# zhuker/lamejs

Measured on NVIDIA H100. Metric: encoded audio seconds/sec (44.1kHz stereo 128kbps CBR), higher is better.
Workload: dtype f64

## Files before the change

### lamejs_b200/csrc/k_quant.cuh

```cuda
#ifndef MP3B200_K_QUANT_CUH
#define MP3B200_K_QUANT_CUH
#include <stddef.h>
#include "mp3_device.cuh"
#include "mp3_tables.h"
#include "k_psy.cuh"

#define Q_LARGE_BITS 100000
#define Q_IXMAX 8206
#define Q_FULL 0xffffffffu

struct GranuleInfoDev {
  int global_gain, part2_3_length, part2_length, big_values, count1, scalefac_compress;
  int table_select[3], region0_count, region1_count, preflag, scalefac_scale, count1table_select, block_type;
  int subblock_gain[4];
  int count1bits, sfbmax, sfbdivide, sfb_lmax, psymax, psy_lmax, sfb_smin, max_nonzero_coeff;
  int scalefac[MP3_SFBMAX];
  int slen[4];
  int part_row;
  int pad_;
  double xrpow_max;
};
struct QuantFrameState {
  int stream, rel_frame;
  int in_old[2], in_step[2];
// ... 868 lines not shown
#pragma unroll 1
    for (int i = 0; i < MP3_SFBMAX; i++) gi->scalefac[i] = 0;
    gi->xrpow_max = 0;
  }
  const Mp3Geo* geo = &T->geo[is_short ? 1 : 0];
  if (lane == 0) wk->geo = geo;
  {
    float4 v[5];
#pragma unroll
    for (int k = 0; k < 5; k++) { const int q = lane + 32 * k; if (q < 144) v[k] = __ldg(reinterpret_cast<const float4*>(xr_g) + q); }
    if (!is_short) {
#pragma unroll
      for (int k = 0; k < 5; k++) { const int q = lane + 32 * k; if (q < 144) reinterpret_cast<float4*>(wk->xr)[q] = v[k]; }
    } else {
#pragma unroll
      for (int k = 0; k < 5; k++) {
        const int q = lane + 32 * k;
        if (q < 144) {
          const short* ro = geo->reorder + 4 * q;
          wk->xr[__ldg(ro + 0)] = v[k].x; wk->xr[__ldg(ro + 1)] = v[k].y; wk->xr[__ldg(ro + 2)] = v[k].z; wk->xr[__ldg(ro + 3)] = v[k].w;
        }
      }
    }
  }
  __syncwarp();
  if (!is_short) {
    const int lo = T->psfb21[0];
    const double lf = (double)T->longfact[21];
    int keep = lo - 1;
#pragma unroll 1
    for (int j = lo + lane; j < 576; j += 32) {
      int g = 0;
      while (g < 5 && j >= T->psfb21[g + 1]) g++;
      double ath21 = ath_ps[g];
      if (lf > 1e-12) ath21 *= lf;
      if (!(fabs((double)wk->xr[j]) < ath21)) keep = j;
    }
    keep = wmax(keep);
    __syncwarp();
#pragma unroll 1
    for (int j = keep + 1 + lane; j < 576; j += 32) wk->xr[j] = 0.0f;
  } else if (lane == 0) {
#pragma unroll 1
    for (int block = 0; block < 3; block++) {
      bool stop = false;
#pragma unroll 1
      for (int g = 5; g >= 0 && !stop; g--) {
        const int start = T->sfb_s[12] * 3 + (T->sfb_s[13] - T->sfb_s[12]) * block + (T->psfb12[g] - T->psfb12[0]);
        const int end = start + (T->psfb12[g + 1] - T->psfb12[g]);
        double ath12 = ath_ps[g];
        if ((double)T->shortfact[12] > 1e-12) ath12 *= (double)T->shortfact[12];
#pragma unroll 1
        for (int j = end - 1; j >= start; j--) {
          if (fabs((double)wk->xr[j]) < ath12) wk->xr[j] = 0.0f;
          else { stop = true; break; }
        }
      }
    }
  }
  __syncwarp();
  {
    float mx = 0.0f, amax = 0.0f;
#pragma unroll 1
    for (int p = lane; p < 288; p += 32) {
      const float2 x = *reinterpret_cast<const float2*>(&wk->xr[2 * p]);
      const double t0 = fabs((double)x.x), t1 = fabs((double)x.y);
      f32s p0, p1; p0 = sqrt(t0 * sqrt(t0)); p1 = sqrt(t1 * sqrt(t1));
      float2 o; o.x = p0.v; o.y = p1.v;
      *reinterpret_cast<float2*>(&wk->xrpow[2 * p]) = o;
      mx = fmaxf(mx, fmaxf(p0.v, p1.v));
      amax = fmaxf(amax, fmaxf((float)t0, (float)t1));
    }
#pragma unroll 1
    for (int o = 16; o > 0; o >>= 1) { mx = fmaxf(mx, __shfl_xor_sync(Q_FULL, mx, o)); amax = fmaxf(amax, __shfl_xor_sync(Q_FULL, amax, o)); }
    bool energy;
    if ((double)amax > 1E-20) energy = true;
    else {
      if (lane == 0) { double sum = 0; for (int i = 0; i <= 575; ++i) sum += fabs((double)wk->xr[i]); wk->scratch[1] = sum > 1E-20; }
      __syncwarp();
      energy = wk->scratch[1] != 0;
      __syncwarp();
    }
    if (lane == 0) gi->xrpow_max = (double)mx;
    __syncwarp();
    if (!energy) {
#pragma unroll 1
      for (int i = lane; i < 576; i += 32) wk->ixw[i] = 0;
      __syncwarp();
      return false;
    }
  }
  const double masking_lower = is_short ? T->masking_lower_short : T->masking_lower_long;
  if (!is_short) {
    if (need_xmin && lane < 21) {
      const int gsfb = lane;
      int j = T->sfb_l[gsfb];
      const int width = wk->geo->width[gsfb];
      double xmin = ath_adjust * (double)T->ath_l[gsfb];
      double en0 = 0.0;
#pragma unroll 1
      for (int l = width >> 1; l > 0; l--) {
        double xa = (double)wk->xr[j] * (double)wk->xr[j]; en0 += xa; j++;
        double xb = (double)wk->xr[j] * (double)wk->xr[j]; en0 += xb; j++;
      }
      const double e = (double)ratio->en_l[gsfb];
      if (e > 0.0) {
        const double x = en0 * (double)ratio->thm_l[gsfb] * masking_lower / e;
        if (xmin < x) xmin = x;
      }
      f32s o; o = xmin * (double)T->longfact[gsfb];
      wk->xmin[gsfb] = o.v;
    }
    int last = -1;
#pragma unroll 1
    for (int i = lane; i < 576; i += 32) if (wk->xr[i] != 0.0f) last = i;
    last = wmax(last);
    int mnz = last + 1;
    if (mnz > 575) mnz = 575;
    if (lane == 0) gi->max_nonzero_coeff = mnz;
  } else {
#pragma unroll 1
    for (int t = lane; need_xmin && t < 36; t += 32) {
      const int sfb = t / 3, b = t - 3 * sfb;
      const int width = wk->geo->width[t];
      int j = 3 * T->sfb_s[sfb] + b * width;
      const double tmpATH = ath_adjust * (double)T->ath_s[sfb];
      double en0 = 0.0;
#pragma unroll 1
      for (int l = width >> 1; l > 0; l--) {
        double xa = (double)wk->xr[j] * (double)wk->xr[j]; en0 += xa; j++;
        double xb = (double)wk->xr[j] * (double)wk->xr[j]; en0 += xb; j++;
      }
      double xmin = tmpATH;
      const double e = (double)ratio->en_s[sfb][b];
      if (e > 0.0) {
        const double x = en0 * (double)ratio->thm_s[sfb][b] * masking_lower / e;
        if (xmin < x) xmin = x;
      }
      f32s o; o = xmin * (double)T->shortfact[sfb];
      wk->xmin[t] = o.v;
    }
    __syncwarp();
    if (need_xmin && lane < 12) {
      f32s* p = reinterpret_cast<f32s*>(&wk->xmin[3 * lane]);
      if ((double)p[0] > (double)p[1]) p[1] += ((double)p[0] - (double)p[1]) * T->decay;
      if ((double)p[1] > (double)p[2]) p[2] += ((double)p[1] - (double)p[2]) * T->decay;
    }
    if (lane == 0) gi->max_nonzero_coeff = 575;
  }
  __syncwarp();
  return true;
}

__device__ __noinline__ void best_scalefac_store_w(GcWork* wk, int* scfsi, const GranuleInfoDev* __restrict__ g0, int gr, int mode_gr) {
  const int lane = LANE;
  GranuleInfoDev* gi = &wk->b;
#pragma unroll 1
  for (int s0 = 0; s0 < gi->sfbmax; s0 += 32) {
    const int sfb = s0 + lane;
    if (sfb < gi->sfbmax) {
      const int j = wk->geo->start[sfb];
      bool any = false;
#pragma unroll 1
      for (int l = 0; l < wk->geo->width[sfb]; l += 2) if (*reinterpret_cast<const unsigned*>(&wk->ixw[j + l]) != 0) { any = true; break; }
      wk->mode[sfb] = any ? 1 : 0;
    }
  }
  __syncwarp();
  const int sfbmax = gi->sfbmax;
  int recalc_w = 0;
  {
    bool z = false;
#pragma unroll 1
    for (int sfb = lane; sfb < sfbmax; sfb += 32) if (!wk->mode[sfb]) { gi->scalefac[sfb] = -2; z = true; }
    if (__any_sync(Q_FULL, z)) recalc_w = -2;
  }
  __syncwarp();
  if (0 == gi->scalefac_scale && 0 == gi->preflag) {
    int sor = 0;
#pragma unroll 1
    for (int sfb = lane; sfb < sfbmax; sfb += 32) { const int v = gi->scalefac[sfb]; if (v > 0) sor |= v; }
    sor = (int)__reduce_or_sync(Q_FULL, (unsigned)sor);
    if (0 == (sor & 1) && sor != 0) {
#pragma unroll 1
      for (int sfb = lane; sfb < sfbmax; sfb += 32) { const int v = gi->scalefac[sfb]; if (v > 0) gi->scalefac[sfb] = v >> 1; }
      __syncwarp();
      if (lane == 0) gi->scalefac_scale = 1;
      recalc_w = 1;
    }
  }
  __syncwarp();
  if (0 == gi->preflag && gi->block_type != BT_SHORT && mode_gr == 2) {
    const bool in = lane >= 11 && lane < 21;
    const int v = in ? gi->scalefac[lane] : 0, pt = pretab_of(lane);
    const bool ok = !in || !(v < pt && v != -2);
    if (__all_sync(Q_FULL, ok)) {
      if (in && v > 0) gi->scalefac[lane] = v - pt;
      __syncwarp();
      if (lane == 0) gi->preflag = 1;
      recalc_w = 1;
    }
  }
  __syncwarp();
  if (lane == 0) {
    int recalc = recalc_w;
#pragma unroll 1
    for (int i = 0; i < 4; i++) scfsi[i] = 0;
    if (gr == 1 && g0->block_type != BT_SHORT && gi->block_type != BT_SHORT) {
      const int* g0sf = g0->scalefac;
      const int band[5] = {0, 6, 11, 16, 21};
      int sfb;
#pragma unroll 1
      for (int i = 0; i < 4; i++) {
#pragma unroll 1
        for (sfb = band[i]; sfb < band[i + 1]; sfb++)
          if (g0sf[sfb] != gi->scalefac[sfb] && gi->scalefac[sfb] >= 0) break;
        if (sfb == band[i + 1]) {
#pragma unroll 1
          for (sfb = band[i]; sfb < band[i + 1]; sfb++) gi->scalefac[sfb] = -1;
          scfsi[i] = 1;
        }
      }
      int s1 = 0, c1 = 0;
#pragma unroll 1
      for (sfb = 0; sfb < 11; sfb++) {
        if (gi->scalefac[sfb] == -1) continue;
        c1++;
        if (s1 < gi->scalefac[sfb]) s1 = gi->scalefac[sfb];
      }
      int s2 = 0, c2 = 0;
#pragma unroll 1
      for (; sfb < 21; sfb++) {
        if (gi->scalefac[sfb] == -1) continue;
        c2++;
        if (s2 < gi->scalefac[sfb]) s2 = gi->scalefac[sfb];
      }
#pragma unroll 1
      for (int i = 0; i < 16; i++) {
        if (s1 < c_slen1_n[i] && s2 < c_slen2_n[i]) {
          const int c = c_slen1_tab[i] * c1 + c_slen2_tab[i] * c2;
          if (gi->part2_length > c) { gi->part2_length = c; gi->scalefac_compress = i; }
        }
      }
      recalc = 0;
    }
    wk->scratch[0] = recalc;
  }
  __syncwarp();
#pragma unroll 1
  for (int sfb = lane; sfb < sfbmax; sfb += 32) if (gi->scalefac[sfb] == -2) gi->scalefac[sfb] = 0;
  __syncwarp();
  const int recalc = wk->scratch[0];
  __syncwarp();
  if (recalc != 0) scale_bitcount_any_w(gi, mode_gr);
}

struct DivScratch {
  unsigned ab[23][7];
  unsigned short cc[23][7];
  unsigned short bmax[23], nesc[23];
  int r0bits[16]; unsigned char r0t[16];
  int cbits[128]; unsigned char ct1[128];
};
static_assert(sizeof(DivScratch) <= 576 * sizeof(float), "DivScratch must fit into the xrpow array");

__device__ __noinline__ int band_stats_w(const Mp3Tables* T, const short* ix, int bigv, DivScratch* ds) {
  const int lane = LANE;
  const unsigned* w32 = reinterpret_cast<const unsigned*>(ix);
  int B = 0;
  while (B < 22 && T->sfb_l[B + 1] <= bigv) B++;
  const int nb = (B < 22 && T->sfb_l[B] < bigv) ? B + 1 : B;
  __syncwarp();
#pragma unroll 1
  for (int b = lane; b < nb; b += 32) {
    const int lo = T->sfb_l[b] >> 1, hi = (b < B ? T->sfb_l[b + 1] : bigv) >> 1;
    unsigned m = 0, ne = 0;
#pragma unroll 1
    for (int p = lo; p < hi; p++) { const unsigned w = w32[p]; m = __vmaxu2(m, w); ne += ((w & 0xffffu) > 14u) + ((w >> 16) > 14u); }
    ds->bmax[b] = (unsigned short)max(m & 0xffffu, m >> 16);
    ds->nesc[b] = (unsigned short)ne;
  }
  __syncwarp();
#pragma unroll 1
  for (int t = lane; t < nb * 7; t += 32) {
    const int b = t / 7, c = t - 7 * b;
    const int mx = ds->bmax[b];
    const int lowc = mx <= 1 ? 0 : (mx <= 3 ? mx - 1 : (mx <= 5 ? 3 : (mx <= 7 ? 4 : (mx <= 15 ? 5 : 6))));
    if (c < lowc) continue;
    const unsigned int* tab = g_cat_tab[c];
    const int lo = T->sfb_l[b] >> 1, hi = (b < B ? T->sfb_l[b + 1] : bigv) >> 1;
    unsigned sa = 0, sb = 0, sc = 0;
#pragma unroll 1
    for (int p = lo; p < hi; p++) {
      const unsigned w = w32[p];
      const unsigned v = __ldg(&tab[min(w & 0xffffu, 15u) * 16 + min(w >> 16, 15u)]);
      sa += v & 0x7ffu; sb += (v >> 11) & 0x7ffu; sc += v >> 22;
    }
    DOMAIN_MISS(DOM_BITSUM_FIELD, sa > 0xffffu || sb > 0xffffu || sc > 0xffffu);
    ds->ab[b][c] = sa | (sb << 16);
    ds->cc[b][c] = (unsigned short)sc;
  }
  __syncwarp();
  return nb;
}

__device__ __forceinline__ int region_from_bands(const DivScratch* ds, int b0, int b1, int* bits) {
  int mx = 0;
#pragma unroll 1
  for (int b = b0; b <= b1; b++) mx = max(mx, (int)ds->bmax[b]);
  if (mx == 0) return 0;
  const RegionClass rc = region_class(mx);
  int sa = 0, sb = 0, sc = 0, ne = 0;
#pragma unroll 1
  for (int b = b0; b <= b1; b++) {
    const unsigned u = ds->ab[b][rc.cat];
    sa += (int)(u & 0xffffu); sb += (int)(u >> 16); sc += ds->cc[b][rc.cat]; ne += ds->nesc[b];
  }
  if (rc.cat == 6) { sa += ne * (int)(rc.lin & 0x7ffu); sb += ne * (int)((rc.lin >> 11) & 0x7ffu); sc = sb; }
  return region_pick(mx, rc, sa, sb, sc, bits);
}

__device__ __noinline__ void divide_init_w(const Mp3Tables* T, DivScratch* ds, int bigv, int* r01_bits, int* r01_div, int* r0_tbl, int* r1_tbl) {
  const int lane = LANE;
  if (lane < 16) {
    int bits0 = -1, t0 = 0;
    if (T->sfb_l[lane + 1] < bigv) { bits0 = 0; t0 = region_from_bands(ds, 0, lane, &bits0); }
    ds->r0bits[lane] = bits0; ds->r0t[lane] = (unsigned char)t0;
  }
  __syncwarp();
#pragma unroll 1
  for (int k = lane; k < 128; k += 32) {
    const int r0 = k >> 3, r1 = k & 7;
    int bits = -1, t1 = 0;
    if (ds->r0bits[r0] >= 0 && r0 + r1 + 2 <= 22 && T->sfb_l[r0 + r1 + 2] < bigv) {
      bits = ds->r0bits[r0];
      t1 = region_from_bands(ds, r0 + 1, r0 + r1 + 1, &bits);
    }
    ds->cbits[k] = bits; ds->ct1[k] = (unsigned char)t1;
  }
  __syncwarp();
  if (lane < 23) {
    const int sidx = lane;
    int best = Q_LARGE_BITS;
#pragma unroll 1
    for (int r0 = 0; r0 < 16; r0++) {
      const int r1 = sidx - r0;
      if (r1 < 0 || r1 > 7) continue;
      const int bits = ds->cbits[r0 * 8 + r1];
      if (bits < 0) continue;
      if (best > bits) { best = bits; r01_div[sidx] = r0; r0_tbl[sidx] = ds->r0t[r0]; r1_tbl[sidx] = ds->ct1[r0 * 8 + r1]; }
    }
    r01_bits[sidx] = best;
  }
  __syncwarp();
}

__device__ __noinline__ void recalc_divide_sub_w(const Mp3Tables* T, GcWork* wk, DivScratch* ds, int nb, const GranuleInfoDev* cod_info2,
                                                 const int* r01_bits, const int* r01_div, const int* r0_tbl, const int* r1_tbl) {
  const int lane = LANE;
  GranuleInfoDev* gi = &wk->b;
  const int bigv = cod_info2->big_values;
  if (lane + 2 <= 22) {
    const int r2 = lane + 2;
    int bits2 = 0, t2 = 0;
    if (T->sfb_l[r2] < bigv) t2 = region_from_bands(ds, r2, nb - 1, &bits2);
    ds->cbits[r2] = bits2; ds->ct1[r2] = (unsigned char)t2;
  }
  __syncwarp();
  int cur = gi->part2_3_length, best_r2 = -1;
  const int c1bits = cod_info2->count1bits;
#pragma unroll 1
  for (int r2 = 2; r2 < 22 + 1; r2++) {
    if (T->sfb_l[r2] >= bigv) break;
    int bits = r01_bits[r2 - 2] + c1bits;
    if (cur <= bits) break;
    bits += ds->cbits[r2];
    if (cur <= bits) continue;
    cur = bits; best_r2 = r2;
  }
  __syncwarp();
  if (best_r2 >= 0) {
    if (cod_info2 != gi) copy_gi_w(gi, cod_info2);
    if (lane == 0) {
      gi->part2_3_length = cur;
      gi->region0_count = r01_div[best_r2 - 2];
      gi->region1_count = best_r2 - 2 - r01_div[best_r2 - 2];
      gi->table_select[0] = r0_tbl[best_r2 - 2];
      gi->table_select[1] = r1_tbl[best_r2 - 2];
      gi->table_select[2] = ds->ct1[best_r2];
    }
    __syncwarp();
  }
}

__device__ __noinline__ void best_huffman_divide_w(const Mp3Tables* T, GcWork* wk) {
  const int lane = LANE;
  GranuleInfoDev* gi = &wk->b;
  GranuleInfoDev* c2 = &wk->w;
  const short* ix = wk->ixw;
  int* r01_bits = reinterpret_cast<int*>(wk->pn_noise_log);
  int* r01_div = reinterpret_cast<int*>(wk->distort);
  int* r0_tbl = wk->pn_step;
  int* r1_tbl = reinterpret_cast<int*>(wk->pn_noise);
  DivScratch* ds = reinterpret_cast<DivScratch*>(wk->xrpow);
  if (gi->block_type == BT_SHORT && T->mode_gr == 1) return;
  copy_gi_w(c2, gi);
  if (gi->block_type == BT_NORM) {
    const int bigv = gi->big_values;
    const int nb = band_stats_w(T, ix, bigv, ds);
    divide_init_w(T, ds, bigv, r01_bits, r01_div, r0_tbl, r1_tbl);
    recalc_divide_sub_w(T, wk, ds, nb, c2, r01_bits, r01_div, r0_tbl, r1_tbl);
  }
  int i = c2->big_values;
  if (i == 0 || (ix[i - 2] | ix[i - 1]) > 1) return;
  i = gi->count1 + 2;
  if (i > 576) return;
  copy_gi_w(c2, gi);
  int a1 = 0, a2 = 0;
  {
    const int top = i, bv = c2->big_values;
    int v1 = 0, v2 = 0, n = 0;
#pragma unroll 1
    for (int q = lane; top - 4 * q > bv; q += 32) {
      const int e = top - 4 * q;
      const int p = ((ix[e - 4] * 2 + ix[e - 3]) * 2 + ix[e - 2]) * 2 + ix[e - 1];
      v1 += __ldg(&g_t32l[p]); v2 += __ldg(&g_t33l[p]); n++;
    }
    a1 = wsum(v1); a2 = wsum(v2);
    i = top - 4 * wsum(n);
  }
  __syncwarp();
  if (lane == 0) {
    c2->count1 = gi->count1 + 2;
    c2->big_values = i;
    c2->count1table_select = 0;
    int a = a1;
    if (a1 > a2) { a = a2; c2->count1table_select = 1; }
    c2->count1bits = a;
  }
  __syncwarp();
  if (a1 > a2) a1 = a2;
  if (c2->block_type == BT_NORM) {
    const int nb2 = band_stats_w(T, ix, i, ds);
    recalc_divide_sub_w(T, wk, ds, nb2, c2, r01_bits, r01_div, r0_tbl, r1_tbl);
  } else {
    int p23 = a1;
    int b1 = T->sfb_l[7 + 1];
    if (b1 > i) b1 = i;
    int t0 = c2->table_select[0], t1 = c2->table_select[1];
    if (b1 > 0) t0 = region_table_w(ix, 0, b1, &p23);
    if (i > b1) t1 = region_table_w(ix, b1, i, &p23);
    __syncwarp();
    if (lane == 0) { c2->part2_3_length = p23; c2->table_select[0] = t0; c2->table_select[1] = t1; }
    __syncwarp();
    if (gi->part2_3_length > c2->part2_3_length) copy_gi_w(gi, c2);
  }
}

__device__ Q_HELPER void put_bits(unsigned int* buf, int pos, unsigned int val, int n) {
  if (n <= 0) return;
  val &= (n >= 32) ? 0xffffffffu : ((1u << n) - 1u);
  const int w = pos >> 5, off = pos & 31;
  const int room = 32 - off;
  if (n <= room) atomicOr(&buf[w], val << (room - n));
  else {
    atomicOr(&buf[w], val >> (n - room));
    atomicOr(&buf[w + 1], val << (32 - (n - room)));
  }
}

#define QNEG(i) (((neg[(i) >> 5] >> ((i) & 31)) & 1u) != 0u)
__device__ __noinline__ void pack_gc_w(const Mp3Tables* T, unsigned int* buf, const GranuleInfoDev* gi, const short* ixq,
                                       const unsigned* neg, int pos) {
  const int lane = LANE;
  if (lane == 0 && T->mode_gr == 1) {
    int p = pos, i = 0;
#pragma unroll 1
    for (int part = 0; part < 4; part++) {
      const int cnt = gi->part_row == 1 ? 9 : (part == 0 ? 6 : 5), sl = gi->slen[part];
#pragma unroll 1
      for (int k = 0; k < cnt; k++, i++) { put_bits(buf, p, (unsigned)max(gi->scalefac[i], 0), sl); p += sl; }
    }
  } else if (lane == 0) {
    const int slen1 = c_slen1_tab[gi->scalefac_compress], slen2 = c_slen2_tab[gi->scalefac_compress];
    int p = pos;
#pragma unroll 1
    for (int sfb = 0; sfb < gi->sfbmax; sfb++) {
      if (gi->scalefac[sfb] == -1) continue;
      const int sl = sfb < gi->sfbdivide ? slen1 : slen2;
      put_bits(buf, p, (unsigned)gi->scalefac[sfb], sl);
      p += sl;
    }
  }
  pos += gi->part2_length;
  const int bigv = gi->big_values;
  int r1s, r2s;
  if (gi->block_type == BT_SHORT) {
    r1s = 3 * T->sfb_s[3];
    if (r1s > bigv) r1s = bigv;
    r2s = bigv;
  } else {
    r1s = T->sfb_l[gi->region0_count + 1];
    r2s = T->sfb_l[gi->region0_count + 1 + gi->region1_count + 1];
    if (r1s > bigv) r1s = bigv;
    if (r2s > bigv) r2s = bigv;
  }
  const int npairs = bigv >> 1;
  const int per = (npairs + 31) >> 5;
  const int p0 = lane * per, p1 = min(npairs, p0 + per);
  int mybits = 0;
#pragma unroll 1
  for (int pass = 0; pass < 2; pass++) {
    int at = 0;
    if (pass == 1) {
      int incl = mybits;
      for (int o = 1; o < 32; o <<= 1) { const int v = __shfl_up_sync(Q_FULL, incl, o); if (lane >= o) incl += v; }
      at = pos + incl - mybits;
    }
#pragma unroll 1
    for (int pr = p0; pr < p1; pr++) {
      const int i = 2 * pr;
      int tb = i < r1s ? gi->table_select[0] : (i < r2s ? gi->table_select[1] : gi->table_select[2]);
      if (tb == 14) tb = 16;
      if (tb == 0) continue;
      const int hx = c_huff_xlen[tb];
      int linbits = hx, xlen = hx;
      int cbits = 0, xbits = 0;
      unsigned ext = 0;
      int x1 = ixq[i], x2 = ixq[i + 1];
      if (x1 != 0) { if (QNEG(i)) ext++; cbits--; }
      if (tb > 15) {
        if (x1 > 14) { ext |= (unsigned)(x1 - 15) << 1; xbits = linbits; x1 = 15; }
        if (x2 > 14) { ext <<= linbits; ext |= (unsigned)(x2 - 15); xbits += linbits; x2 = 15; }
        xlen = 16;
      }
      if (x2 != 0) { ext <<= 1; if (QNEG(i + 1)) ext++; cbits--; }
      const int idx = x1 * xlen + x2;
      xbits -= cbits;
      cbits += __ldg(&g_huff_len[c_huff_off[tb] + idx]);
      if (pass == 0) mybits += cbits + xbits;
      else {
        put_bits(buf, at, __ldg(&g_huff_code[c_huff_off[tb] + idx]), cbits);
        put_bits(buf, at + cbits, ext, xbits);
        at += cbits + xbits;
      }
    }
  }
  const int big_bits = wsum(mybits);
  pos += big_bits;
  const int nquads = (gi->count1 - bigv) >> 2;
  const int perq = (nquads + 31) >> 5;
  const int q0 = lane * perq, q1 = min(nquads, q0 + perq);
  const int tb = gi->count1table_select + 32;
  mybits = 0;
#pragma unroll 1
  for (int pass = 0; pass < 2; pass++) {
    int at = 0;
    if (pass == 1) {
      int incl = mybits;
      for (int o = 1; o < 32; o <<= 1) { const int v = __shfl_up_sync(Q_FULL, incl, o); if (lane >= o) incl += v; }
      at = pos + incl - mybits;
    }
#pragma unroll 1
    for (int q = q0; q < q1; q++) {
      const int i = bigv + 4 * q;
      int huffbits = 0, p = 0;
      if (ixq[i] != 0) { p += 8; if (QNEG(i)) huffbits++; }
      if (ixq[i + 1] != 0) { p += 4; huffbits *= 2; if (QNEG(i + 1)) huffbits++; }
      if (ixq[i + 2] != 0) { p += 2; huffbits *= 2; if (QNEG(i + 2)) huffbits++; }
      if (ixq[i + 3] != 0) { p++; huffbits *= 2; if (QNEG(i + 3)) huffbits++; }
      const int len = __ldg(&g_huff_len[c_huff_off[tb] + p]);
      if (pass == 0) mybits += len;
      else { put_bits(buf, at, (unsigned)huffbits + __ldg(&g_huff_code[c_huff_off[tb] + p]), len); at += len; }
    }
  }
  __syncwarp();
}

__device__ __forceinline__ void put_header_bits(unsigned int* buf, int pos, int val, int n) {
  while (n > 0) {
    const int k = min(n, 8 - (pos & 7));
    n -= k;
    const unsigned byte = ((unsigned)(val >> n) << (8 - (pos & 7) - k)) & 0xffu;
    const int b = pos >> 3;
    atomicOr(&buf[b >> 2], byte << (24 - 8 * (b & 3)));
    pos += k;
  }
}

__device__ __noinline__ void pack_sideinfo(const Mp3Tables* T, unsigned int* buf, const GranuleInfoDev* __restrict__ fin,
                                           const int* scfsi, int padding) {
  int p = 0;
#define WH(v, n) do { put_header_bits(buf, p, (int)(v), (n)); p += (n); } while (0)
  const int nch = T->nch;
  WH(T->mpeg25 ? 0xffe : 0xfff, 12); WH(T->version, 1); WH(4 - 3, 2); WH(1, 1);
  WH(T->bitrate_index, 4); WH(T->samplerate_index, 2); WH(padding, 1); WH(0, 1);
  WH(T->mono ? 3 : 0, 2); WH(0, 2); WH(0, 1); WH(1, 1); WH(0, 2);
  if (T->version == 1) {
    WH(0, 9);
    WH(0, nch == 2 ? 3 : 5);
#pragma unroll 1
    for (int ch = 0; ch < nch; ch++) for (int b = 0; b < 4; b++) WH(scfsi[ch * 4 + b], 1);
  } else {
    WH(0, 8);
    WH(0, nch);
  }
#pragma unroll 1
  for (int gr = 0; gr < T->mode_gr; gr++) for (int ch = 0; ch < nch; ch++) {
    const GranuleInfoDev* gi = &fin[gr * nch + ch];
    WH(gi->part2_3_length + gi->part2_length, 12);
    WH(gi->big_values / 2, 9);
    WH(gi->global_gain, 8);
    WH(gi->scalefac_compress, T->version == 1 ? 4 : 9);
    int ts0 = gi->table_select[0], ts1 = gi->table_select[1], ts2 = gi->table_select[2];
    if (ts0 == 14) ts0 = 16;
    if (ts1 == 14) ts1 = 16;
    if (gi->block_type != BT_NORM) {
      WH(1, 1); WH(gi->block_type, 2); WH(0, 1);
      WH(ts0, 5); WH(ts1, 5);
      WH(gi->subblock_gain[0], 3); WH(gi->subblock_gain[1], 3); WH(gi->subblock_gain[2], 3);
    } else {
      WH(0, 1);
      if (ts2 == 14) ts2 = 16;
      WH(ts0, 5); WH(ts1, 5); WH(ts2, 5);
      WH(gi->region0_count, 4); WH(gi->region1_count, 3);
    }
    if (T->version == 1) WH(gi->preflag, 1);
    WH(gi->scalefac_scale, 1); WH(gi->count1table_select, 1);
  }
#undef WH
}

__device__ __forceinline__ int granule_budget(int nch, int mean_bits, int gr, int used0, int used1, int ch) {
  int tbits = mean_bits;
  if (gr == 1) {
    const int resv = -(used0 + (nch == 2 ? used1 : 0)) + mean_bits;
    if (resv * 10 > 0) tbits += resv;
  }
  double t = (double)tbits / nch;
  if (t > 4095) t = 4095;
  int targ = (int)t;
  const int bits = targ * nch;
  if (bits > 7680) { targ = targ * 7680; targ = (int)((double)targ / bits); }
  (void)ch;
  return targ;
}

#ifndef Q_WARPS
#define Q_WARPS 4
#endif
#ifndef Q_BLOCKS_PER_SM
#define Q_BLOCKS_PER_SM 7
#endif
#define Q_THREADS (32 * Q_WARPS)

__device__ __forceinline__ int next_task(int* counter) {
  int t = 0;
  if (LANE == 0) t = atomicAdd(counter, 1);
  return __shfl_sync(Q_FULL, t, 0);
}
template <int STRIDE = (int)sizeof(WarpShared)>
__device__ __forceinline__ WarpShared* warp_shared() {
  extern __shared__ __align__(16) unsigned char smem_raw[];
  return reinterpret_cast<WarpShared*>(smem_raw + (threadIdx.x >> 5) * STRIDE);
}
__device__ __forceinline__ void gi_init_w(GranuleInfoDev* gi, const GcPrep* __restrict__ pr) {
  __syncwarp();
  int* w = reinterpret_cast<int*>(gi);
#pragma unroll 1
  for (int i = LANE; i < (int)(sizeof(GranuleInfoDev) / 4); i += 32) w[i] = 0;
  __syncwarp();
  if (LANE == 0) {
    const int bt = pr->block_type;
    const bool is_short = bt == BT_SHORT;
    gi->global_gain = 210; gi->block_type = bt;
    gi->sfb_lmax = is_short ? 0 : 21; gi->sfb_smin = is_short ? 0 : 12; gi->psy_lmax = is_short ? 0 : 21;
    gi->psymax = is_short ? 36 : 21; gi->sfbmax = is_short ? 36 : 21; gi->sfbdivide = is_short ? 18 : 11;
    gi->max_nonzero_coeff = pr->mnz; gi->xrpow_max = pr->xrpow_max;
  }
  __syncwarp();
}
__device__ __forceinline__ void copy_row16_w(void* dst, const void* src, int nbytes) {
  __syncwarp();
  const int n = nbytes >> 4;
  int4 v[5];
#pragma unroll
  for (int k = 0; k < 5; k++) { const int i = LANE + 32 * k; if (i < n) v[k] = reinterpret_cast<const int4*>(src)[i]; }
#pragma unroll
  for (int k = 0; k < 5; k++) { const int i = LANE + 32 * k; if (i < n) reinterpret_cast<int4*>(dst)[i] = v[k]; }
  __syncwarp();
}
struct FrameGeom { int z, f, padding, frame_bytes, mean_bits; long long kabs; };
__device__ __forceinline__ FrameGeom frame_geom(const Mp3Tables* T, const StreamDesc* streams, const QuantFrameState* q) {
  FrameGeom g;
  g.z = q->stream; g.f = q->rel_frame;
  g.kabs = (long long)streams[g.z].frame0 + g.f;
  g.padding = (int)(pad_count(g.kabs, T->frac_SpF, T->samplerate) - pad_count(g.kabs - 1, T->frac_SpF, T->samplerate));
  g.frame_bytes = T->frame_bytes_nopad + g.padding;
  g.mean_bits = (8 * g.frame_bytes - T->sideinfo_len * 8) / T->mode_gr;
  return g;
}

__global__ void __launch_bounds__(Q_THREADS, Q_BLOCKS_PER_SM)
k_q_prepare(const Mp3Tables* __restrict__ T, const StreamDesc* __restrict__ streams, const float* __restrict__ xr,
            const PsyRatioDev* __restrict__ ratio, const signed char* __restrict__ bt_final, const double* __restrict__ ath_q,
            const QuantFrameState* __restrict__ qs, float* __restrict__ xrq, float* __restrict__ xrpow_g, unsigned* __restrict__ neg_g,
            GcPrep* __restrict__ prep,
            int nframes, int* __restrict__ counter) {
  WarpShared* ws = warp_shared();
  GcWork* wk = &ws->wk;
  const int lane = LANE, nch = T->nch;
  const int G = T->mode_gr;
  const int ntasks = nframes * G * nch;
#pragma unroll 1
  for (int t = next_task(counter); t < ntasks; t = next_task(counter)) {
    const int frow = t / (G * nch), rem = t - frow * G * nch, gr = rem / nch, ch = rem - gr * nch;
    const QuantFrameState* q = qs + frow;
    const int z = q->stream, f = q->rel_frame;
    const StreamDesc& sd = streams[z];
    const double ath_adjust = ath_q[frow];
    const size_t urow = (size_t)sd.unit_base + G * f + gr, gidx = urow * nch + ch;
    const int bt = bt_final[urow * 2 + ch];
    const PsyRatioDev* rt = ratio + ((size_t)sd.unit_base + z + G * f + gr) * nch + ch;
    __syncwarp();
    if (lane < 6) ws->ath[lane] = ath_adjust_dev(ath_adjust, (double)(bt == BT_SHORT ? T->ath_psfb12[lane] : T->ath_psfb21[lane]), T->ath_floor);
    __syncwarp();
    const bool have = gc_prepare_w(T, wk, ws->ath, xr + gidx * 576, bt, rt, ath_adjust);
    copy_row16_w(xrq + gidx * 576, wk->xr, 2304);
    {
      unsigned mine = 0;
#pragma unroll 1
      for (int k = 0; k < 18; k++) { const unsigned m = __ballot_sync(Q_FULL, wk->xr[lane + 32 * k] < 0.0f); if (lane == k) mine = m; }
      if (lane < 18) neg_g[gidx * 18 + lane] = mine;
    }
    copy_row16_w(xrpow_g + gidx * 576, wk->xrpow, 2304);
    GcPrep* pr = prep + gidx;
#pragma unroll 1
    for (int i = lane; i < MP3_SFBMAX; i += 32) pr->xmin[i] = wk->xmin[i];
    if (lane == 0) { pr->have = have ? 1 : 0; pr->mnz = wk->b.max_nonzero_coeff; pr->block_type = bt; pr->xrpow_max = wk->b.xrpow_max; }
  }
}

__global__ void __launch_bounds__(Q_THREADS, Q_SLIM_BLOCKS)
k_q_search(const Mp3Tables* __restrict__ T, const StreamDesc* __restrict__ streams, QuantFrameState* __restrict__ qs,
           GranuleInfoDev* __restrict__ ginfo, short* __restrict__ l3enc, const float* __restrict__ xrpow_g,
           const GcPrep* __restrict__ prep, int gr, const int* __restrict__ list, const int* __restrict__ count_ptr, int count_direct,
           int revalidate, int* __restrict__ counter, int* __restrict__ list2, int* __restrict__ count2,
           int* __restrict__ list3, int* __restrict__ count3) {
  WarpShared* ws = warp_shared<Q_STRIDE_NOXR>();
  GcWork* wk = &ws->wk;
  const int lane = LANE, nch = T->nch;
  const int ntasks = (count_ptr ? *count_ptr : count_direct) * nch;
#pragma unroll 1
  for (int t = next_task(counter); t < ntasks; t = next_task(counter)) {
    const int wi = t / nch, ch = t - wi * nch;
    const int frow = list ? list[wi] : wi;
    QuantFrameState* q = qs + frow;
    const int flags = revalidate ? q->redo : 0;
    if (revalidate == 3 && (flags & Q_R0_ANY)) continue;
    if (revalidate && gr == 1 && !(flags & (Q_R0_ANY | Q_R1S(ch)))) continue;
    const FrameGeom fg = frame_geom(T, streams, q);
    const StreamDesc& sd = streams[fg.z];
    const size_t urow = (size_t)sd.unit_base + T->mode_gr * fg.f + gr, gidx = urow * nch + ch;
    const int targ = granule_budget(nch, fg.mean_bits, gr, q->used0[0], q->used0[1], ch);
    int ov = gr == 0 ? q->in_old[ch] : q->bs_gain0[ch];
    int cs = gr == 0 ? q->in_step[ch] : q->bs_step0[ch];
    const GcPrep* pr = prep + gidx;
    const bool have = pr->have != 0;
    gi_init_w(&wk->b, pr);
    if (lane == 0) wk->geo = &T->geo[pr->block_type == BT_SHORT ? 1 : 0];
    unsigned long long h = 0;
    if (have) {
      copy_row16_w(wk->xrpow, xrpow_g + gidx * 576, 2304);
      QSTAT(revalidate ? 12 + gr : 11);
      bin_search_w(T, wk, targ, &ov, &cs, revalidate ? 2 + 2 * gr : 0);
      h = gi_hash(&wk->b);
    } else {
      __syncwarp();
#pragma unroll 1
      for (int i = lane; i < 288; i += 32) reinterpret_cast<unsigned*>(wk->ixw)[i] = 0;
      __syncwarp();
    }
    bool store;
    if (!revalidate) {
      store = true;
      if (gr == 0 && fg.f != 0 && T->mode_gr == 2) cs = Q_SPEC_GR1_STEP;
      if (lane == 0) {
        q->bs_hash[gr][ch] = h;
        if (gr == 0) { q->bs_gain0[ch] = ov; q->bs_step0[ch] = cs; }
        if (gr == T->mode_gr - 1) { q->out_old[ch] = ov; q->out_step[ch] = cs; }
      }
    } else if (gr == 0) {
      store = ov != q->bs_gain0[ch] || h != q->bs_hash[0][ch];
      const bool step_changed = cs != q->bs_step0[ch];
      __syncwarp();
      if (lane == 0) {
        int old = -1;
        if (T->mode_gr == 1) { q->out_old[ch] = ov; q->out_step[ch] = cs; }
        if (store) {
          q->bs_gain0[ch] = ov; q->bs_step0[ch] = cs; q->bs_hash[0][ch] = h; old = atomicOr(&q->redo, Q_R0(ch));
          if ((old & Q_R0_ANY) == 0) list3[atomicAdd(count3, 1)] = frow;
        } else if (step_changed && T->mode_gr == 2) { q->bs_step0[ch] = cs; old = atomicOr(&q->redo, Q_R1S(ch)); }
        if (old == 0) list2[atomicAdd(count2, 1)] = frow;
      }
    } else {
      store = (flags & Q_R0_ANY) || ov != q->out_old[ch] || h != q->bs_hash[1][ch];
      __syncwarp();
      if (lane == 0) {
        q->out_step[ch] = cs;
        if (store) { q->out_old[ch] = ov; q->bs_hash[1][ch] = h; atomicOr(&q->redo, Q_R1(ch)); }
      }
    }
    if (store) {
      copy_row16_w(l3enc + gidx * 576, wk->ixw, 1152);
      copy_gi_w(&ginfo[gidx], &wk->b);
    }
  }
}

__global__ void __launch_bounds__(Q_THREADS, Q_BLOCKS_PER_SM)
k_q_outer(const Mp3Tables* __restrict__ T, const StreamDesc* __restrict__ streams, QuantFrameState* __restrict__ qs,
          GranuleInfoDev* __restrict__ ginfo, short* __restrict__ l3enc, const float* __restrict__ xrq,
          const float* __restrict__ xrpow_g, const GcPrep* __restrict__ prep, int gr, const int* __restrict__ list,
          const int* __restrict__ count_ptr, int count_direct, int revalidate, int* __restrict__ counter) {
  WarpShared* ws = warp_shared();
  GcWork* wk = &ws->wk;
  const int lane = LANE, nch = T->nch;
  const int ntasks = (count_ptr ? *count_ptr : count_direct) * nch;
#pragma unroll 1
  for (int t = next_task(counter); t < ntasks; t = next_task(counter)) {
    const int wi = t / nch, ch = t - wi * nch;
#ifdef Q_REVERSE
    const int frow = list ? list[wi] : (ntasks / nch - 1 - wi);
#else
    const int frow = list ? list[wi] : wi;
#endif
    QuantFrameState* q = qs + frow;
    if (revalidate == 1 && !(q->redo & (gr == 0 ? Q_R0(ch) : Q_R1(ch)))) continue;
    if (revalidate == -1 && (q->redo & Q_R0_ANY)) continue;
    if (revalidate > 0) QSTAT(14);
    const FrameGeom fg = frame_geom(T, streams, q);
    const StreamDesc& sd = streams[fg.z];
    const size_t urow = (size_t)sd.unit_base + T->mode_gr * fg.f + gr, gidx = urow * nch + ch;
    const int targ = granule_budget(nch, fg.mean_bits, gr, q->used0[0], q->used0[1], ch);
    const GcPrep* pr = prep + gidx;
    const bool have = pr->have != 0;
    short* const ixrow = l3enc + gidx * 576;
    __syncwarp();
    if (lane == 0) { wk->geo = &T->geo[pr->block_type == BT_SHORT ? 1 : 0]; wk->ixg = ixrow; }
    copy_gi_w(&wk->b, &ginfo[gidx]);
    copy_row16_w(wk->ixw, ixrow, 1152);
#ifdef Q_TASKSTAT
    const long long ts_t0 = clock64();
    const int ts_gain = wk->b.global_gain, ts_bits = wk->b.part2_3_length;
#endif
    if (have) {
      copy_row16_w(wk->xr, xrq + gidx * 576, 2304);
      copy_row16_w(wk->xrpow, xrpow_g + gidx * 576, 2304);
#pragma unroll 1
      for (int i = lane; i < MP3_SFBMAX; i += 32) wk->xmin[i] = pr->xmin[i];
      __syncwarp();
      outer_loop_w(T, wk, targ);
    }
#ifdef Q_TASKSTAT
    if (lane == 0 && revalidate <= 0 && gidx < (1u << 16)) {
      int* r = g_taskstat[gidx];
      r[0] = (int)((clock64() - ts_t0) >> 6); r[1] = gr; r[2] = wk->b.max_nonzero_coeff; r[3] = wk->b.block_type;
      r[4] = ts_gain; r[5] = ts_bits; r[6] = targ; r[7] = wk->b.global_gain;
    }
#endif
    copy_gi_w(&ginfo[gidx], &wk->b);
    copy_row16_w(ixrow, wk->ixw, 1152);
  }
}

__global__ void __launch_bounds__(Q_THREADS, Q_SLIM_BLOCKS)
k_q_finish(const Mp3Tables* __restrict__ T, const StreamDesc* __restrict__ streams, QuantFrameState* __restrict__ qs,
           GranuleInfoDev* __restrict__ ginfo, short* __restrict__ l3enc, int gr, const int* __restrict__ list,
           const int* __restrict__ count_ptr, int count_direct, int revalidate, int* __restrict__ counter) {
  WarpShared* ws = warp_shared<Q_STRIDE_NOXR>();
  GcWork* wk = &ws->wk;
  const int lane = LANE, nch = T->nch;
  const int ntasks = (count_ptr ? *count_ptr : count_direct) * nch;
#pragma unroll 1
  for (int t = next_task(counter); t < ntasks; t = next_task(counter)) {
    const int wi = t / nch, ch = t - wi * nch;
    const int frow = list ? list[wi] : wi;
    QuantFrameState* q = qs + frow;
    if (revalidate == 1 && !(q->redo & (gr == 0 ? Q_R0(ch) : Q_R1(ch)))) continue;
    if (revalidate == -1 && (q->redo & Q_R0_ANY)) continue;
    const StreamDesc& sd = streams[q->stream];
    const size_t urow = (size_t)sd.unit_base + T->mode_gr * q->rel_frame + gr, gidx = urow * nch + ch;
    short* const ixrow = l3enc + gidx * 576;
    copy_gi_w(&wk->b, &ginfo[gidx]);
    copy_row16_w(wk->ixw, ixrow, 1152);
    if (lane == 0) wk->geo = &T->geo[wk->b.block_type == BT_SHORT ? 1 : 0];
    __syncwarp();
    best_scalefac_store_w(wk, ws->scfsi, gr == 1 ? &ginfo[gidx - nch] : nullptr, gr, T->mode_gr);
    best_huffman_divide_w(T, wk);
    copy_gi_w(&ginfo[gidx], &wk->b);
    if (gr == 0) { if (lane == 0) q->used0[ch] = wk->b.part2_3_length + wk->b.part2_length; }
    else if (lane < 4) q->scfsi[ch][lane] = ws->scfsi[lane];
  }
}

struct __align__(16) PackShared {
  unsigned int bits[368];
  short ix[576];
  unsigned neg[20];
  GranuleInfoDev gi;
  int scfsi[8];
};
__global__ void __launch_bounds__(Q_THREADS)
k_q_pack(const Mp3Tables* __restrict__ T, const StreamDesc* __restrict__ streams, QuantFrameState* __restrict__ qs,
         const GranuleInfoDev* __restrict__ ginfo, const short* __restrict__ l3enc, const unsigned* __restrict__ neg_g,
         const int* __restrict__ list, const int* __restrict__ count_ptr, int count_direct, int revalidate,
         int* __restrict__ counter, uint8_t* __restrict__ out, int* __restrict__ over_budget) {
  extern __shared__ __align__(16) unsigned char smem_raw[];
  PackShared* ps = reinterpret_cast<PackShared*>(smem_raw) + (threadIdx.x >> 5);
  const int lane = LANE, nch = T->nch;
  const int ntasks = count_ptr ? *count_ptr : count_direct;
#pragma unroll 1
  for (int t = next_task(counter); t < ntasks; t = next_task(counter)) {
    const int frow = list ? list[t] : t;
    QuantFrameState* q = qs + frow;
    if (revalidate && !(q->redo & (Q_R0_ANY | Q_R1_ANY))) continue;
    if (revalidate) QSTAT(5);
    const FrameGeom fg = frame_geom(T, streams, q);
    const StreamDesc& sd = streams[fg.z];
    const size_t g0 = ((size_t)sd.unit_base + T->mode_gr * fg.f) * nch;
    int used = 0;
#pragma unroll 1
    for (int k = 0; k < T->mode_gr * nch; k++) used += ginfo[g0 + k].part2_3_length + ginfo[g0 + k].part2_length;
    const bool over = used > 8 * (fg.frame_bytes - T->sideinfo_len);
    if (lane == 0 && over != (q->valid == 2)) atomicAdd(over_budget, over ? 1 : -1);
    if (over) { if (lane == 0) q->valid = 2; continue; }
    __syncwarp();
#pragma unroll 1
    for (int i = lane; i < 368; i += 32) ps->bits[i] = 0;
    if (lane < 8) ps->scfsi[lane] = q->scfsi[lane >> 2][lane & 3];
    __syncwarp();
    int pos = 8 * T->sideinfo_len;
#pragma unroll 1
    for (int k = 0; k < T->mode_gr * nch; k++) {
      copy_gi_w(&ps->gi, &ginfo[g0 + k]);
      copy_row16_w(ps->ix, l3enc + (g0 + k) * 576, 1152);
      if (lane < 18) ps->neg[lane] = neg_g[(g0 + k) * 18 + lane];
      __syncwarp();
      pack_gc_w(T, ps->bits, &ps->gi, ps->ix, ps->neg, pos);
      pos += ps->gi.part2_3_length + ps->gi.part2_length;
      __syncwarp();
    }
    if (lane == 0) {
      pack_sideinfo(T, ps->bits, ginfo + g0, ps->scfsi, fg.padding);
      int remaining = 8 * fg.frame_bytes - pos;
      const unsigned char tag[10] = {0x4c, 0x41, 0x4d, 0x45, 3, 0, 9, 8, 0, 4};
      int k = 0;
      for (; k < 4 && remaining >= 8; k++) { put_bits(ps->bits, pos, tag[k], 8); pos += 8; remaining -= 8; }
      if (remaining >= 32) for (; k < 10 && remaining >= 8; k++) { put_bits(ps->bits, pos, tag[k], 8); pos += 8; remaining -= 8; }
    }
    __syncwarp();
    const long long off = sd.out_base + (long long)fg.f * T->frame_bytes_nopad +
                          (pad_count(fg.kabs - 1, T->frac_SpF, T->samplerate) - pad_count((long long)sd.frame0 - 1, T->frac_SpF, T->samplerate));
    uint8_t* dst = out + off;
#pragma unroll 1
    for (int i = lane; i < fg.frame_bytes; i += 32) dst[i] = (uint8_t)(ps->bits[i >> 2] >> (24 - 8 * (i & 3)));
    if (lane == 0) q->valid = 1;
  }
}

__global__ void k_qstate_init(const StreamDesc* __restrict__ streams, int nstreams, QuantFrameState* __restrict__ qs) {
  const int z = blockIdx.y;
  const StreamDesc sd = streams[z];
  const int f = blockIdx.x * blockDim.x + threadIdx.x;
  if (f >= sd.nframes) return;
  QuantFrameState* q = qs + sd.frame_base + f;
  q->stream = z; q->rel_frame = f; q->valid = 0; q->redo = 0;
#pragma unroll 1
  for (int c = 0; c < 2; c++) {
    q->in_old[c] = f == 0 ? sd.old_value[c] : Q_SPEC_START;
    q->in_step[c] = f == 0 ? sd.current_step[c] : Q_SPEC_STEP;
    q->out_old[c] = q->out_step[c] = 0;
    q->used0[c] = 0; q->bs_gain0[c] = q->bs_step0[c] = 0;
    for (int b = 0; b < 4; b++) q->scfsi[c][b] = 0;
  }
}

__global__ void k_qstate_verify(const StreamDesc* __restrict__ streams, QuantFrameState* __restrict__ qs, long long nframes,
                                int* __restrict__ list, int* __restrict__ counter, int predict_step) {
  const long long r = (long long)blockIdx.x * blockDim.x + threadIdx.x;
  if (r >= nframes) return;
  QuantFrameState* q = qs + r;
  if (q->rel_frame == 0) return;
  const QuantFrameState* p = q - 1;
  int pstep[2] = {p->out_step[0], p->out_step[1]};
  if (predict_step && p->rel_frame != 0) {
    const QuantFrameState* pp = p - 1;
#pragma unroll 1
    for (int c = 0; c < 2; c++) pstep[c] = (pp->out_old[c] - p->out_old[c] >= 4) ? 4 : 2;
  }
  bool same = true;
#pragma unroll 1
  for (int c = 0; c < 2; c++) if (q->in_old[c] != p->out_old[c] || q->in_step[c] != pstep[c]) same = false;
  if (!same) {
#pragma unroll 1
    for (int c = 0; c < 2; c++) { q->in_old[c] = p->out_old[c]; q->in_step[c] = pstep[c]; }
    q->redo = 0;
    list[atomicAdd(counter, 1)] = (int)r;
  }
}

__global__ void k_qstate_commit(StreamDesc* __restrict__ streams, int nstreams, const QuantFrameState* __restrict__ qs) {
  const int z = blockIdx.x * blockDim.x + threadIdx.x;
  if (z >= nstreams) return;
  StreamDesc& sd = streams[z];
  if (sd.nframes <= 0) return;
  const QuantFrameState* q = qs + sd.frame_base + sd.nframes - 1;
#pragma unroll 1
  for (int c = 0; c < 2; c++) { sd.old_value[c] = q->out_old[c]; sd.current_step[c] = q->out_step[c]; }
}

__global__ void k_qstate_loop_cond(cudaGraphConditionalHandle loop, int* __restrict__ count, int* __restrict__ st, int max_passes) {
  const int n = *count;
  int passes = st[2];
  bool more = n != 0;
  if (more) passes++;
  if (passes > max_passes) { st[1] = 1; *count = 0; more = false; }
  st[2] = passes;
  if (passes > st[0]) st[0] = passes;
  cudaGraphSetConditional(loop, more ? 1u : 0u);
}

struct QuantBuffers {
  const float* xr; const PsyRatioDev* ratio; const signed char* bt; const double* ath_q;
  QuantFrameState* qs; GranuleInfoDev* ginfo; short* l3enc; float* xrq; float* xrpow; unsigned* neg; GcPrep* prep;
  int* over_budget;
  int* list; int* counter;
};
#define Q_NCOUNTERS 256
#define Q_REPAIR_BLOCKS 16
enum { QE_START, QE_PREP, QE_S0, QE_O0, QE_F0, QE_S1, QE_MID, QE_O1, QE_F1, QE_PK, QE_COUNT };

struct QuantLoop {
  cudaStream_t capture = nullptr;
  int* st = nullptr;
  cudaGraphExec_t exec = nullptr;
};

static int quant_run(const Mp3Tables* dT, const Mp3Tables& hT, StreamDesc* d_streams, int S, int nstreams_with_frames, int max_frames, long long F,
                     const QuantBuffers& B, cudaStream_t st_main, cudaStream_t st_repair, cudaEvent_t ev_fork, cudaEvent_t ev_join,
                     cudaEvent_t ev_pass1, cudaEvent_t* evq, int* evq_pred, int* passes_out, std::atomic<long long>* launches,
                     QuantLoop* dloop = nullptr) {
  cudaStream_t st = st_main;
  static std::mutex attr_mu;
  static bool attr_done[64] = {};
  int dev = 0, sms = 132;
  cudaGetDevice(&dev);
  cudaDeviceGetAttribute(&sms, cudaDevAttrMultiProcessorCount, dev);
  const size_t smem = sizeof(WarpShared) * Q_WARPS, smem_slim = (size_t)Q_STRIDE_NOXR * Q_WARPS, smem_pack = sizeof(PackShared) * Q_WARPS;
  {
    std::lock_guard<std::mutex> lk(attr_mu);
    if (dev < 64 && !attr_done[dev]) {
      if (cudaFuncSetAttribute(k_q_prepare, cudaFuncAttributeMaxDynamicSharedMemorySize, (int)smem) != cudaSuccess) return -100;
      if (cudaFuncSetAttribute(k_q_search, cudaFuncAttributeMaxDynamicSharedMemorySize, (int)smem_slim) != cudaSuccess) return -100;
      if (cudaFuncSetAttribute(k_q_outer, cudaFuncAttributeMaxDynamicSharedMemorySize, (int)smem) != cudaSuccess) return -100;
      if (cudaFuncSetAttribute(k_q_finish, cudaFuncAttributeMaxDynamicSharedMemorySize, (int)smem_slim) != cudaSuccess) return -100;
      if (cudaFuncSetAttribute(k_q_pack, cudaFuncAttributeMaxDynamicSharedMemorySize, (int)smem_pack) != cudaSuccess) return -100;
      attr_done[dev] = true;
    }
  }
  if (F <= 0) { *passes_out = 0; return 0; }
  const int nch = hT.nch;
  int next_counter = Q_NCOUNTERS;
  auto fresh_counter = [&]() -> int* {
    if (next_counter >= Q_NCOUNTERS) { cudaMemsetAsync(B.counter + 3, 0, sizeof(int) * (Q_NCOUNTERS - 3), st); next_counter = 3; }
    return B.counter + next_counter++;
  };
  auto grid_for = [&](long long tasks, int per_sm) -> int {
    long long g = (tasks + Q_WARPS - 1) / Q_WARPS, cap = (long long)sms * per_sm;
    if (g > cap) g = cap;
    return (int)(g < 1 ? 1 : g);
  };
  {
    dim3 g((max_frames + 127) / 128, S);
    k_qstate_init<<<g, 128, 0, st>>>(d_streams, S, B.qs);
    (*launches)++;
  }
  for (int i = 0; i < QE_COUNT; i++) evq_pred[i] = -1;
  int last_slot = -1;
  auto mark = [&](int slot) { cudaEventRecord(evq[slot], st); evq_pred[slot] = last_slot; last_slot = slot; };
  int* const prep_counter = fresh_counter();
  mark(QE_START);
  k_q_prepare<<<grid_for(F * hT.mode_gr * nch, Q_BLOCKS_PER_SM), Q_THREADS, smem, st>>>(dT, d_streams, B.xr, B.ratio, B.bt, B.ath_q, B.qs, B.xrq, B.xrpow, B.neg,
                                                                              B.prep, (int)F, prep_counter);
  mark(QE_PREP);
  (*launches)++;
  int* const list1 = B.list;
  int* const list2 = B.list + (F + 1);
  int* const list3 = B.list + 2 * (F + 1);
  auto search = [&](int gr, const int* list, const int* cptr, long long count, int reval) {
    k_q_search<<<grid_for(count * nch, Q_SLIM_BLOCKS), Q_THREADS, smem_slim, st>>>(dT, d_streams, B.qs, B.ginfo, B.l3enc, B.xrpow, B.prep, gr, list, cptr, (int)count,
                                                                             reval, fresh_counter(), list2, B.counter + 1, list3, B.counter + 2);
    (*launches)++;
  };
  int reserve_blocks = 0;
  auto finish = [&](int gr, const int* list, const int* cptr, long long count, int reval) {
    k_q_finish<<<max(1, grid_for(count * nch, Q_SLIM_BLOCKS) - reserve_blocks), Q_THREADS, smem_slim, st>>>(dT, d_streams, B.qs, B.ginfo, B.l3enc, gr, list, cptr, (int)count, reval, fresh_counter());
    (*launches)++;
  };
  auto outer = [&](int gr, const int* list, const int* cptr, long long count, int reval) {
    k_q_outer<<<max(1, grid_for(count * nch, Q_BLOCKS_PER_SM) - reserve_blocks), Q_THREADS, smem, st>>>(dT, d_streams, B.qs, B.ginfo, B.l3enc, B.xrq, B.xrpow, B.prep, gr, list, cptr, (int)count,
                                                                            reval, fresh_counter());
    (*launches)++;
  };
  auto outer_finish = [&](int gr, long long count, int reval, int slot_o, int slot_f) {
    outer(gr, nullptr, nullptr, count, reval); mark(slot_o);
    finish(gr, nullptr, nullptr, count, reval); mark(slot_f);
  };
  auto pack = [&](const int* list, const int* cptr, long long count, int reval) {
    k_q_pack<<<grid_for(count, 9), Q_THREADS, smem_pack, st>>>(dT, d_streams, B.qs, B.ginfo, B.l3enc, B.neg, list, cptr, (int)count, reval, fresh_counter(), nullptr, B.over_budget);
    (*launches)++;
  };
  auto verify = [&](int predict_step = 0) {
    cudaMemsetAsync(B.counter, 0, 3 * sizeof(int), st);
    k_qstate_verify<<<(int)((F + 255) / 256), 256, 0, st>>>(d_streams, B.qs, F, list1, B.counter, predict_step);
    (*launches)++;
  };
  const int G = hT.mode_gr;
  const bool speculated = F > nstreams_with_frames;
  search(0, nullptr, nullptr, F, 0); mark(QE_S0);
  if (G == 2) {
    outer_finish(0, F, 0, QE_O0, QE_F0);
    search(1, nullptr, nullptr, F, 0); mark(QE_S1);
  }
  bool forked = false;
  if (Q_SPEC_FOLD && speculated) {
    verify(G == 1 ? 1 : 0);
    search(0, list1, B.counter, F, 1);
    if (G == 2) {
      search(1, list2, B.counter + 1, F, 3);
      int* const c0 = fresh_counter(); int* const c1 = fresh_counter(); int* const c2 = fresh_counter();
      int* const c3 = fresh_counter(); int* const c4 = fresh_counter();
      cudaEventRecord(ev_fork, st_main);
      cudaStreamWaitEvent(st_repair, ev_fork, 0);
      const int gq = Q_REPAIR_BLOCKS, gs = Q_REPAIR_BLOCKS;
      const int* cp = B.counter + 2;
      k_q_outer<<<gq, Q_THREADS, smem, st_repair>>>(dT, d_streams, B.qs, B.ginfo, B.l3enc, B.xrq, B.xrpow, B.prep, 0, list3, cp, (int)F, 1, c0);
      k_q_finish<<<gs, Q_THREADS, smem_slim, st_repair>>>(dT, d_streams, B.qs, B.ginfo, B.l3enc, 0, list3, cp, (int)F, 1, c1);
      k_q_search<<<gs, Q_THREADS, smem_slim, st_repair>>>(dT, d_streams, B.qs, B.ginfo, B.l3enc, B.xrpow, B.prep, 1, list3, cp, (int)F, 1, c2, list2, B.counter + 1,
                                                          list3, B.counter + 2);
      k_q_outer<<<gq, Q_THREADS, smem, st_repair>>>(dT, d_streams, B.qs, B.ginfo, B.l3enc, B.xrq, B.xrpow, B.prep, 1, list3, cp, (int)F, 2, c3);
      k_q_finish<<<gs, Q_THREADS, smem_slim, st_repair>>>(dT, d_streams, B.qs, B.ginfo, B.l3enc, 1, list3, cp, (int)F, 2, c4);
      cudaEventRecord(ev_join, st_repair);
      (*launches) += 5;
      forked = true;
    }
  }
  mark(QE_MID);
  if (G == 2) {
    reserve_blocks = forked ? Q_REPAIR_BLOCKS : 0;
    outer_finish(1, F, forked ? -1 : 0, QE_O1, QE_F1);
    reserve_blocks = 0;
    if (forked) cudaStreamWaitEvent(st_main, ev_join, 0);
  } else {
    outer_finish(0, F, 0, QE_O0, QE_F0);
  }
  pack(nullptr, nullptr, F, 0); mark(QE_PK);
  if (cudaEventRecord(ev_pass1, st) != cudaSuccess) return -100;
  int passes = 2;
  auto revalidate = [&](const int* count1, long long count) {
    search(0, list1, count1, count, 1);
    outer(0, list2, B.counter + 1, count, 1);
    finish(0, list2, B.counter + 1, count, 1);
    if (G == 2) {
      search(1, list2, B.counter + 1, count, 1);
      outer(1, list2, B.counter + 1, count, 1);
      finish(1, list2, B.counter + 1, count, 1);
    }
    pack(list2, B.counter + 1, count, 1);
  };
  if (dloop && speculated) {
    if (!dloop->exec) {
      cudaGraph_t g = nullptr;
      cudaGraphConditionalHandle cond;
      cudaGraphNode_t reset, loop;
      cudaMemsetParams mp = {};
      mp.dst = dloop->st + 2; mp.value = 2; mp.elementSize = sizeof(int); mp.width = 1; mp.height = 1;
      cudaGraphNodeParams cp = {};
      cp.type = cudaGraphNodeTypeConditional;
      if (cudaGraphCreate(&g, 0) != cudaSuccess) return -100;
      bool ok = cudaGraphConditionalHandleCreate(&cond, g, 1, cudaGraphCondAssignDefault) == cudaSuccess &&
                cudaGraphAddMemsetNode(&reset, g, nullptr, 0, &mp) == cudaSuccess;
      cp.conditional.handle = cond; cp.conditional.type = cudaGraphCondTypeWhile; cp.conditional.size = 1;
      ok = ok && cudaGraphAddNode(&loop, g, &reset, 1, &cp) == cudaSuccess;
      cudaGraph_t body = ok ? cp.conditional.phGraph_out[0] : nullptr;
      if (ok && cudaStreamBeginCaptureToGraph(dloop->capture, body, nullptr, nullptr, 0, cudaStreamCaptureModeThreadLocal) == cudaSuccess) {
        std::atomic<long long> captured{0};
        std::atomic<long long>* const counted = launches;
        launches = &captured;
        st = dloop->capture;
        next_counter = Q_NCOUNTERS;
        verify();
        k_qstate_loop_cond<<<1, 1, 0, st>>>(cond, B.counter, dloop->st, max_frames + 3);
        revalidate(B.counter, F);
        st = st_main;
        launches = counted;
        cudaGraph_t captured_body = nullptr;
        ok = cudaStreamEndCapture(dloop->capture, &captured_body) == cudaSuccess && captured_body == body &&
             cudaGraphInstantiate(&dloop->exec, g, 0) == cudaSuccess;
      } else {
        ok = false;
      }
      cudaGraphDestroy(g);
      if (!ok) { dloop->exec = nullptr; return -100; }
    }
    if (cudaGraphLaunch(dloop->exec, st) != cudaSuccess) return -100;
    (*launches)++;
  }
  for (; speculated && !dloop;) {
    verify();
    int h_count = 0;
    if (cudaMemcpyAsync(&h_count, B.counter, sizeof(int), cudaMemcpyDeviceToHost, st) != cudaSuccess) return -100;
    if (cudaStreamSynchronize(st) != cudaSuccess) return -100;
    if (h_count == 0) break;
    revalidate(nullptr, h_count);
    passes++;
    if (passes > max_frames + 3) return -100;
  }
  k_qstate_commit<<<(S + 63) / 64, 64, 0, st>>>(d_streams, S, B.qs);
  (*launches)++;
  *passes_out = passes;
  return 0;
}

#endif
```

Baseline: 60840.

## Inline Huffman divide helpers, recompute only last band, raise finish occupancy, fuse commit

```diff
diff --git a/lamejs_b200/csrc/k_quant.cuh b/lamejs_b200/csrc/k_quant.cuh
--- a/lamejs_b200/csrc/k_quant.cuh
+++ b/lamejs_b200/csrc/k_quant.cuh
@@ -1044,7 +1044,7 @@
   return true;
 }
 
-__device__ __noinline__ void best_scalefac_store_w(GcWork* wk, int* scfsi, const GranuleInfoDev* __restrict__ g0, int gr, int mode_gr) {
+__device__ __forceinline__ void best_scalefac_store_w(GcWork* wk, int* scfsi, const GranuleInfoDev* __restrict__ g0, int gr, int mode_gr) {
   const int lane = LANE;
   GranuleInfoDev* gi = &wk->b;
 #pragma unroll 1
@@ -1156,15 +1156,16 @@
 };
 static_assert(sizeof(DivScratch) <= 576 * sizeof(float), "DivScratch must fit into the xrpow array");
 
-__device__ __noinline__ int band_stats_w(const Mp3Tables* T, const short* ix, int bigv, DivScratch* ds) {
+__device__ __forceinline__ int band_stats_w(const Mp3Tables* T, const short* ix, int bigv, DivScratch* ds, bool last_only = false) {
   const int lane = LANE;
   const unsigned* w32 = reinterpret_cast<const unsigned*>(ix);
   int B = 0;
   while (B < 22 && T->sfb_l[B + 1] <= bigv) B++;
   const int nb = (B < 22 && T->sfb_l[B] < bigv) ? B + 1 : B;
-  __syncwarp();
-#pragma unroll 1
-  for (int b = lane; b < nb; b += 32) {
+  const int b0 = last_only ? B : 0;
+  __syncwarp();
+#pragma unroll 1
+  for (int b = b0 + lane; b < nb; b += 32) {
     const int lo = T->sfb_l[b] >> 1, hi = (b < B ? T->sfb_l[b + 1] : bigv) >> 1;
     unsigned m = 0, ne = 0;
 #pragma unroll 1
@@ -1174,8 +1175,8 @@
   }
   __syncwarp();
 #pragma unroll 1
-  for (int t = lane; t < nb * 7; t += 32) {
-    const int b = t / 7, c = t - 7 * b;
+  for (int t = lane; t < (nb - b0) * 7; t += 32) {
+    const int b = b0 + t / 7, c = t - 7 * (b - b0);
     const int mx = ds->bmax[b];
     const int lowc = mx <= 1 ? 0 : (mx <= 3 ? mx - 1 : (mx <= 5 ? 3 : (mx <= 7 ? 4 : (mx <= 15 ? 5 : 6))));
     if (c < lowc) continue;
@@ -1212,7 +1213,7 @@
   return region_pick(mx, rc, sa, sb, sc, bits);
 }
 
-__device__ __noinline__ void divide_init_w(const Mp3Tables* T, DivScratch* ds, int bigv, int* r01_bits, int* r01_div, int* r0_tbl, int* r1_tbl) {
+__device__ __forceinline__ void divide_init_w(const Mp3Tables* T, DivScratch* ds, int bigv, int* r01_bits, int* r01_div, int* r0_tbl, int* r1_tbl) {
   const int lane = LANE;
   if (lane < 16) {
     int bits0 = -1, t0 = 0;
@@ -1247,8 +1248,8 @@
   __syncwarp();
 }
 
-__device__ __noinline__ void recalc_divide_sub_w(const Mp3Tables* T, GcWork* wk, DivScratch* ds, int nb, const GranuleInfoDev* cod_info2,
-                                                 const int* r01_bits, const int* r01_div, const int* r0_tbl, const int* r1_tbl) {
+__device__ __forceinline__ void recalc_divide_sub_w(const Mp3Tables* T, GcWork* wk, DivScratch* ds, int nb, const GranuleInfoDev* cod_info2,
+                                                    const int* r01_bits, const int* r01_div, const int* r0_tbl, const int* r1_tbl) {
   const int lane = LANE;
   GranuleInfoDev* gi = &wk->b;
   const int bigv = cod_info2->big_values;
@@ -1285,7 +1286,7 @@
   }
 }
 
-__device__ __noinline__ void best_huffman_divide_w(const Mp3Tables* T, GcWork* wk) {
+__device__ __forceinline__ void best_huffman_divide_w(const Mp3Tables* T, GcWork* wk) {
   const int lane = LANE;
   GranuleInfoDev* gi = &wk->b;
   GranuleInfoDev* c2 = &wk->w;
@@ -1333,7 +1334,7 @@
   __syncwarp();
   if (a1 > a2) a1 = a2;
   if (c2->block_type == BT_NORM) {
-    const int nb2 = band_stats_w(T, ix, i, ds);
+    const int nb2 = band_stats_w(T, ix, i, ds, true);
     recalc_divide_sub_w(T, wk, ds, nb2, c2, r01_bits, r01_div, r0_tbl, r1_tbl);
   } else {
     int p23 = a1;
@@ -1545,6 +1546,7 @@
 #define Q_BLOCKS_PER_SM 7
 #endif
 #define Q_THREADS (32 * Q_WARPS)
+#define Q_FINISH_BLOCKS 10
 
 __device__ __forceinline__ int next_task(int* counter) {
   int t = 0;
@@ -1766,7 +1768,7 @@
   }
 }
 
-__global__ void __launch_bounds__(Q_THREADS, Q_SLIM_BLOCKS)
+__global__ void __launch_bounds__(Q_THREADS, Q_FINISH_BLOCKS)
 k_q_finish(const Mp3Tables* __restrict__ T, const StreamDesc* __restrict__ streams, QuantFrameState* __restrict__ qs,
            GranuleInfoDev* __restrict__ ginfo, short* __restrict__ l3enc, int gr, const int* __restrict__ list,
            const int* __restrict__ count_ptr, int count_direct, int revalidate, int* __restrict__ counter) {
@@ -1902,7 +1904,9 @@
   }
 }
 
-__global__ void k_qstate_commit(StreamDesc* __restrict__ streams, int nstreams, const QuantFrameState* __restrict__ qs) {
+__global__ void k_qstate_commit(StreamDesc* __restrict__ streams, int nstreams, const QuantFrameState* __restrict__ qs,
+                                const int* __restrict__ pending) {
+  if (pending && *pending != 0) return;
   const int z = blockIdx.x * blockDim.x + threadIdx.x;
   if (z >= nstreams) return;
   StreamDesc& sd = streams[z];
@@ -1997,7 +2001,7 @@
   };
   int reserve_blocks = 0;
   auto finish = [&](int gr, const int* list, const int* cptr, long long count, int reval) {
-    k_q_finish<<<max(1, grid_for(count * nch, Q_SLIM_BLOCKS) - reserve_blocks), Q_THREADS, smem_slim, st>>>(dT, d_streams, B.qs, B.ginfo, B.l3enc, gr, list, cptr, (int)count, reval, fresh_counter());
+    k_q_finish<<<max(1, grid_for(count * nch, Q_FINISH_BLOCKS) - reserve_blocks), Q_THREADS, smem_slim, st>>>(dT, d_streams, B.qs, B.ginfo, B.l3enc, gr, list, cptr, (int)count, reval, fresh_counter());
     (*launches)++;
   };
   auto outer = [&](int gr, const int* list, const int* cptr, long long count, int reval) {
@@ -2109,8 +2113,13 @@
     if (cudaGraphLaunch(dloop->exec, st) != cudaSuccess) return -100;
     (*launches)++;
   }
+  auto commit = [&](const int* pending) {
+    k_qstate_commit<<<(S + 63) / 64, 64, 0, st>>>(d_streams, S, B.qs, pending);
+    (*launches)++;
+  };
   for (; speculated && !dloop;) {
     verify();
+    commit(B.counter);
     int h_count = 0;
     if (cudaMemcpyAsync(&h_count, B.counter, sizeof(int), cudaMemcpyDeviceToHost, st) != cudaSuccess) return -100;
     if (cudaStreamSynchronize(st) != cudaSuccess) return -100;
@@ -2119,8 +2128,7 @@
     passes++;
     if (passes > max_frames + 3) return -100;
   }
-  k_qstate_commit<<<(S + 63) / 64, 64, 0, st>>>(d_streams, S, B.qs);
-  (*launches)++;
+  if (!speculated || dloop) commit(nullptr);
   *passes_out = passes;
   return 0;
 }
```

Measured after the change: 61500 (median of 6 runs). No clear change (+1.1%).
